# BGU-CS-VIL/DPMMSubClusters.jl

Hardware: NVIDIA B200
Metric: gibbs_iters_per_sec (higher is better)
Workload: dtype f32

## Files before the change

dpmmsubclusters.jl_b200/csrc/kernels_gauss_tc2.cuh:

```cuda
#pragma once
#include "tcgen05.cuh"
#include "kernels_gauss.cuh"
#include "kernels_stats.cuh"

#define T2_TILE 128
#define T2_PRODUCERS(D) ((D) == 32 ? 128 : 64)
#define T2_THREADS(D) (320 + T2_PRODUCERS(D))
#define T2_CMAX 8
#define T2_R 8
#define T2_DELTA 30.0f
#define T2_MAX_K 256
#define T2_COOP_MAX 12
#define T2_NS32 4

struct GaussTc2Args {
  const float* x;
  int64_t n;
  int K, KS, nch, n0;
  const int32_t* perm;
  const int32_t* seg_off;
  int nkeys;
  const float* wpiv;
  const float* wscr;
  const float* wbias;
// ... 489 lines not shown
            if constexpr (D == 64) {
              tc::tmem_ld32(taddr, v);
              tc::tmem_ld32(taddr + 32, v1);
              tc::tmem_ld_wait();
              qp = gauss_tc_screen_q(v) + gauss_tc_screen_q(v1);
            } else {
              tc::tmem_ld32(taddr, v);
              tc::tmem_ld32(taddr + 32, v1);
              tc::tmem_ld_wait();
              qp = gauss_tc_screen_q(v);
            }
            const float2 cf = ccfro[key];
            const float e = xnorm * cf.y;
            float sq;
            asm("sqrt.approx.ftz.f32 %0, %1;" : "=f"(sq) : "f"(fmaxf(qp, 0.f)));
            const float dr = fmaf(1.01f * sq, e, fmaf(0.5f * e, e, 0.01f));
            const float rt = fmaf(-0.5f, qp, cf.x);
            weird = !(fabsf(rt) < CUDART_INF_F) || !(dr < CUDART_INF_F);
            thr = (rt - dr) - T2_DELTA;
            A4 = 4.0816f * (0.01f - thr);
            A42 = f2_pack(A4, A4);
            col = D;
            if constexpr (D == 32) {
              uint32_t h = screen4(v1, 0);
              if ((unsigned)key < 4u) h &= ~(1u << key);
              if (h) append(h, 0);
              b0 = 1;
            }
          }
          for (; b0 < nb; b0 += 2) {
            uint32_t v[32], v1[32];
            tc::tmem_ld32(taddr + col + b0 * 32, v);
            if (b0 + 1 < nb) tc::tmem_ld32(taddr + col + b0 * 32 + 32, v1);
            tc::tmem_ld_wait();
            uint32_t h = screen4(v, c * 16 + b0 * 4);
            if (b0 + 1 < nb) h |= screen4(v1, c * 16 + b0 * 4 + 4) << 4;
            const int k0 = kbase + b0 * 4;
            if ((unsigned)(key - k0) < 8u) h &= ~(1u << (key - k0));
            if (h) append(h, k0);
          }
          tc::tc_fence_before();
          tc::mbar_arrive(&tempty[g * 2 + b]);
        }
        bool multi = valid && !weird && cnt > 0 && cnt < T2_CMAX;
        bool ovf = valid && (weird || cnt >= T2_CMAX);
        if (multi) {
          int j = cnt;
          while (j > 0 && mylist[j - 1] > key) {
            mylist[j] = mylist[j - 1];
            --j;
          }
          mylist[j] = (uint16_t)key;
          ++cnt;
        }
        if (__any_sync(0xffffffffu, multi)) {
          const int mine = multi ? cnt : 0;
          int inc = mine;
#pragma unroll
          for (int o = 1; o < 32; o <<= 1) {
            const int t = __shfl_up_sync(0xffffffffu, inc, o);
            if (lane >= o) inc += t;
          }
          const int total = __shfl_sync(0xffffffffu, inc, 31), off = inc - mine;
          uint16_t* wpairs = pairs + wq * 32 * T2_CMAX;
          for (int j = 0; j < mine; ++j) wpairs[off + j] = (uint16_t)((row << 3) | j);
          __syncwarp();
          if (total <= T2_COOP_MAX) {
            for (int p = 0; p < total; ++p) {
              const int pr = wpairs[p], prow = pr >> 3, slot = pr & 7;
              const int k = lists[prow * T2_CMAX + slot];
              const int32_t pidx = __ldg(a.perm + w.pos + prow);
              const float q = gauss_tc2_exact_q_coop<D>(a.urows + (size_t)k * D * D, a.mu + (size_t)k * D, a.x + (size_t)pidx * D, lane);
              if (lane == 0) {
                const float2 cf = cfin[k];
                rl[prow * T2_CMAX + slot] = gauss_finish(cf.x, q, cf.y);
                ++ncand_total;
              }
            }
          } else {
            for (int p = lane; p < total; p += 32) {
              const int pr = wpairs[p], prow = pr >> 3, slot = pr & 7;
              const int k = lists[prow * T2_CMAX + slot];
              const int32_t pidx = __ldg(a.perm + w.pos + prow);
              const float q = gauss_tc2_exact_q_row<D>(a.urows + (size_t)k * D * D, a.mu + (size_t)k * D, a.x + (size_t)pidx * D);
              const float2 cf = cfin[k];
              rl[prow * T2_CMAX + slot] = gauss_finish(cf.x, q, cf.y);
              ++ncand_total;
            }
          }
          __syncwarp();
        }
        tc::mbar_arrive(&empty[s]);
        if (valid) {
          int lab = key;
          if (multi) {
            bool bad = false;
            for (int j = 0; j < cnt; ++j) bad |= (myrl[j] != myrl[j]);
            if (bad) {
              ovf = true;
            } else if (a.final_iter) {
              float bv = -CUDART_INF_F;
              lab = mylist[0];
              for (int j = 0; j < cnt; ++j)
                if (myrl[j] > bv) {
                  bv = myrl[j];
                  lab = mylist[j];
                }
            } else {
              const double u = dpmm_uniform(a.u_inj, idx, a.seed, DPMM_STREAM_LABEL, a.call, (uint64_t)(a.goff + idx));
              lab = gauss_tc2_draw_list(mylist, myrl, cnt, K, u);
            }
          } else if (!ovf) {
            if (a.u_inj != nullptr && lab > 0 && !a.final_iter && a.u_inj[idx] == 0.0) lab = 0;
          }
          if (ovf) {
            a.ovf_list[atomicAdd(a.ovf_count, 1)] = idx;
          } else {
            a.labels[idx] = lab;
            atomicAdd(&hs[lab], 1);
          }
          ++npts_total;
        }
      }
      {
#pragma unroll
        for (int o = 16; o > 0; o >>= 1) {
          npts_total += __shfl_xor_sync(0xffffffffu, npts_total, o);
          ncand_total += __shfl_xor_sync(0xffffffffu, ncand_total, o);
        }
        if (lane == 0 && a.stats != nullptr) {
          atomicAdd(&a.stats[0], npts_total);
          atomicAdd(&a.stats[1], ncand_total);
        }
      }
    } else {
      const int t64 = tid - 320;
      constexpr int CPR = D / 4;
      constexpr int RS = T2_PRODUCERS(D) / CPR;
      constexpr int NJ = T2_TILE / RS;
      const int c = t64 % CPR, r0 = t64 / CPR;
      T2Walk wl, wc;
      t2_walk_init(wl, seq);
      wc = wl;
      int ckey = -1;
      float4 cen = make_float4(0.f, 0.f, 0.f, 0.f);
      int32_t idx[NJ];
      auto load_idx = [&]() {
#pragma unroll
        for (int j = 0; j < NJ; ++j) {
          const int p = wl.pos + r0 + RS * j;
          idx[j] = p < wl.end ? __ldg(a.perm + p) : -1;
        }
      };
      auto issue = [&](int s) {
        uint8_t* dst0 = stage0 + (size_t)s * L.stage_bytes + (c >> 3) * 16384;
#pragma unroll
        for (int j = 0; j < NJ; ++j) {
          const int r = r0 + RS * j;
          const bool ok = idx[j] >= 0;
          cp_async16(dst0 + r * 128 + (((c & 7) ^ (r & 7)) << 4), a.x + (size_t)(ok ? idx[j] : 0) * D + 4 * c, ok ? 16 : 0);
        }
      };
      load_idx();
#pragma unroll
      for (int q = 0; q < PF; ++q) {
        if (q < nt) {
          issue(q % NS);
          t2_advance(wl, seq);
          if (q + 1 < nt) load_idx();
        }
        cp_async_commit();
      }
      for (int li = 0; li < nt; ++li) {
        cp_async_wait_group<PF - 1>();
        {
          const int key = min(wc.key, K - 1);
          if (key != ckey) {
            ckey = key;
            cen = __ldg(reinterpret_cast<const float4*>(a.mu + (size_t)key * D) + c);
          }
          uint8_t* base = stage0 + (size_t)(li % NS) * L.stage_bytes + (c >> 3) * 16384;
          const int nrow = wc.end - wc.pos;
#pragma unroll
          for (int j = 0; j < NJ; ++j) {
            const int r = r0 + RS * j;
            float4* q = reinterpret_cast<float4*>(base + r * 128 + (((c & 7) ^ (r & 7)) << 4));
            float4 v = *q;
            if (r < nrow) {
              v.x -= cen.x; v.y -= cen.y; v.z -= cen.z; v.w -= cen.w;
              *q = v;
            }
          }
          t2_advance(wc, seq);
        }
        tc::fence_proxy_async();
        tc::mbar_arrive(&full[li % NS]);
        const int nx = li + PF;
        if (nx < nt) {
          tc::mbar_wait(&empty[nx % NS], ((nx / NS) & 1) ^ 1);
          issue(nx % NS);
          t2_advance(wl, seq);
          if (nx + 1 < nt) load_idx();
        }
        cp_async_commit();
      }
    }
  }
  tc::tc_fence_before();
  __syncthreads();
  if (warp == 1) tc::tmem_dealloc(tmem_base, 512);
  for (int k = tid; k < K; k += T2_THREADS(D))
    if (hs[k] != 0) atomicAdd(&a.hist[k], hs[k]);
}

struct GaussListArgs {
  const float* x;
  int K;
  const int32_t* list;
  const int32_t* count;
  const float* urows;
  const float* mu;
  const float* cst;
  const float* logw;
  int32_t* labels;
  int32_t* hist;
  const double* u_inj;
  uint64_t seed;
  uint32_t call;
  int64_t goff;
  int final_iter;
  int32_t* stats;
  int32_t* zero_next;
  int32_t* ticket;
  int scan_k;
  int32_t* seg_off;
  int32_t* scat_cursor;
  int32_t* lr_cursor;
};

template <int D>
__global__ void __launch_bounds__(256) gauss_label_list_kernel(const GaussListArgs a) {
  extern __shared__ float gl_rs[];
  const int lane = threadIdx.x & 31, wl = threadIdx.x >> 5;
  const int nlist = *a.count;
  if (a.zero_next != nullptr && blockIdx.x == 0 && threadIdx.x < 4) a.zero_next[threadIdx.x] = 0;
  float* rs = gl_rs + (size_t)wl * a.K;
  for (int e = blockIdx.x * 8 + wl; e < nlist; e += gridDim.x * 8) {
    const int32_t idx = a.list[e];
    const float* xr = a.x + (size_t)idx * D;
    for (int k = lane; k < a.K; k += 32) {
      const float q = gauss_tc2_exact_q_impl<D>(a.urows + (size_t)k * D * D, a.mu + (size_t)k * D,
                                                [&](int c) { return __ldg(reinterpret_cast<const float4*>(xr) + c); });
      rs[k] = gauss_finish(__ldg(a.cst + 3 * k), q, __ldg(a.logw + k));
    }
    __syncwarp();
    if (lane == 0) {
      int lab;
      if (a.final_iter) {
        lab = dpmm_draw_argmax(rs, 1, a.K);
      } else {
        const double u = dpmm_uniform(a.u_inj, idx, a.seed, DPMM_STREAM_LABEL, a.call, (uint64_t)(a.goff + idx));
        lab = dpmm_draw_inverse_cdf(rs, 1, a.K, u);
      }
      a.labels[idx] = lab;
      atomicAdd(a.hist + lab, 1);
      if (a.stats != nullptr) atomicAdd(&a.stats[1], a.K);
    }
    __syncwarp();
  }
  if (a.ticket != nullptr) {
    __shared__ int last_block;
    __shared__ int wtot[8];
    __threadfence();
    __syncthreads();
    if (threadIdx.x == 0) last_block = atomicAdd(a.ticket, 1) == (int)gridDim.x - 1;
    __syncthreads();
    if (last_block) {
      __threadfence();
      int carry = 0;
      for (int k0 = 0; k0 < a.scan_k; k0 += 256) {
        const int k = k0 + (int)threadIdx.x;
        const int v = k < a.scan_k ? __ldcg(a.hist + k) : 0;
        int inc = v;
#pragma unroll
        for (int o = 1; o < 32; o <<= 1) {
          const int t = __shfl_up_sync(0xffffffffu, inc, o);
          if (lane >= o) inc += t;
        }
        if (lane == 31) wtot[wl] = inc;
        __syncthreads();
        int before = 0, total = 0;
#pragma unroll
        for (int w = 0; w < 8; ++w) {
          before += w < wl ? wtot[w] : 0;
          total += wtot[w];
        }
        const int excl = carry + before + inc - v;
        if (k < a.scan_k) {
          a.seg_off[k] = excl;
          a.scat_cursor[k] = excl;
          a.lr_cursor[2 * k] = excl;
          a.lr_cursor[2 * k + 1] = excl + v;
        }
        carry += total;
        __syncthreads();
      }
      if (threadIdx.x == 0) {
        a.seg_off[a.scan_k] = carry;
        *a.ticket = 0;
      }
    }
  }
}
```

dpmmsubclusters.jl_b200/csrc/kernels_stats.cuh:

```cuda
#pragma once
#include "common.cuh"

struct StatsItem {
  int32_t key;
  int32_t begin;
  int32_t end;
};

#ifndef DPMM_TEMPLATES_ONLY
__global__ void stats_worklist_kernel(const int32_t* __restrict__ seg_off, const int32_t* __restrict__ lr_cursor,
                                      const uint8_t* __restrict__ wanted, int K, int chunk, StatsItem* items,
                                      int32_t* n_items, int32_t* next_item) {
  extern __shared__ int sc[];
  const int tid = threadIdx.x;
  for (int key = tid; key < 2 * K; key += blockDim.x) {
    const int k = key >> 1;
    int len = 0;
    if (wanted == nullptr || wanted[k]) {
      const int mid = lr_cursor[2 * k];
      len = (key & 1) ? seg_off[k + 1] - mid : mid - seg_off[k];
    }
    sc[key] = (len + chunk - 1) / chunk;
  }
  __syncthreads();
  if (tid == 0) {
    int run = 0;
    for (int key = 0; key < 2 * K; ++key) {
      const int c = sc[key];
      sc[key] = run;
      run += c;
    }
    *n_items = run;
    *next_item = 0;
  }
  __syncthreads();
  for (int key = tid; key < 2 * K; key += blockDim.x) {
    const int k = key >> 1;
    if (wanted != nullptr && !wanted[k]) continue;
    const int mid = lr_cursor[2 * k];
    const int b = (key & 1) ? mid : seg_off[k];
    const int e = (key & 1) ? seg_off[k + 1] : mid;
    int o = sc[key];
    for (int s = b; s < e; s += chunk) items[o++] = StatsItem{key, s, min(e, s + chunk)};
  }
}

#endif

template <int EP>
__device__ __forceinline__ void warp_transpose_reduce(float (&v)[EP], int lane) {
  static_assert(EP % 32 == 0, "EP must be a multiple of 32");
  int h = EP / 2;
#pragma unroll
  for (int s = 0; s < 5; ++s) {
    const int off = 16 >> s;
    const bool up = (lane & off) != 0;
#pragma unroll
    for (int e = 0; e < EP / 2; ++e) {
      if (e < h) {
        const float send = up ? v[e] : v[e + h];
        const float keep = up ? v[e + h] : v[e];
        v[e] = keep + __shfl_xor_sync(0xffffffffu, send, off);
      }
    }
    h >>= 1;
  }
}
template <int EP>
__device__ __forceinline__ int warp_transpose_entry(int lane, int j) {
  int e = j, h = EP / 2;
#pragma unroll
  for (int s = 0; s < 5; ++s) {
    if (lane & (16 >> s)) e += h;
    h >>= 1;
  }
  return e;
}

template <int D>
struct StatsCfg {
  static constexpr int BS = (D <= 8) ? D : 8;
  static constexpr int BSQ = (BS + 1) & ~1;
  static constexpr int NB = (D + BS - 1) / BS;
  static constexpr int NU = NB * (NB + 1) / 2;
  static constexpr int DPAD = NB * BS + (BSQ - BS);
  static constexpr bool VEC = (BS % 4 == 0);
  static constexpr int DS = VEC ? 4 * ((DPAD / 4) | 1) : ((DPAD & 1) ? DPAD : DPAD + 1);
  static constexpr int E = BS * BSQ;
  static constexpr int EP = (E + 31) / 32 * 32;
  static constexpr int G = (NU + 15) / 16;
  static constexpr int WPG = (NU + G - 1) / G;
  static constexpr int NS = (WPG >= 8) ? 1 : (8 / WPG);
  static constexpr int WARPS = WPG * NS;
  static constexpr int R = (NS >= 8) ? 2 : 4;
  static constexpr int TPTS = 32 * NS * R;
  static constexpr int STAGES = 4;
  static constexpr int MAX_CHUNK = 2048;
  static constexpr int SMEM_BYTES = STAGES * TPTS * DS * 4 + MAX_CHUNK * 4;
  static constexpr int MIN_CTAS = (WARPS * 32 <= 320) ? 2 : 1;
};

struct StatsArgs {
  const float* x;
  int D;
  const int32_t* perm2;
  const StatsItem* items;
  const int32_t* n_items;
  int32_t* next_item;
  double* acc;
  int rec;
};

__device__ __forceinline__ void cp_async16(void* smem_dst, const void* gmem_src, int src_bytes) {
  const unsigned d = (unsigned)__cvta_generic_to_shared(smem_dst);
  asm volatile("cp.async.cg.shared.global [%0], [%1], 16, %2;" ::"r"(d), "l"(gmem_src), "r"(src_bytes) : "memory");
}
__device__ __forceinline__ void cp_async4(void* smem_dst, const void* gmem_src, int src_bytes) {
  const unsigned d = (unsigned)__cvta_generic_to_shared(smem_dst);
  asm volatile("cp.async.ca.shared.global [%0], [%1], 4, %2;" ::"r"(d), "l"(gmem_src), "r"(src_bytes) : "memory");
}
__device__ __forceinline__ void cp_async_commit() { asm volatile("cp.async.commit_group;" ::: "memory"); }
__device__ __forceinline__ void cp_async_wait_all() { asm volatile("cp.async.wait_group 0;" ::: "memory"); }
template <int N>
__device__ __forceinline__ void cp_async_wait_group() { asm volatile("cp.async.wait_group %0;" ::"n"(N) : "memory"); }

template <int D>
__global__ void __launch_bounds__(StatsCfg<D>::WARPS * 32, StatsCfg<D>::MIN_CTAS)
niw_stats_kernel(const StatsArgs a) {
  using C = StatsCfg<D>;
  constexpr int BS = C::BS, BSQ = C::BSQ, NQ = C::BSQ / 2;
  extern __shared__ __align__(16) float xs_all[];
  int32_t* sidx = reinterpret_cast<int32_t*>(xs_all + C::STAGES * C::TPTS * C::DS);
  __shared__ int s_item;
  const int tid = threadIdx.x, lane = tid & 31, warp = tid >> 5;
  const int slice = warp / C::WPG;
  for (int e = tid; e < C::STAGES * C::TPTS * C::DS; e += blockDim.x) xs_all[e] = 0.f;

  auto prefetch = [&](const StatsItem& item, int t0, int buf) {
    float* xs = xs_all + buf * C::TPTS * C::DS;
    const int tn = min(C::TPTS, item.end - t0);
    const int32_t* ix = sidx + (t0 - item.begin);
    if constexpr (D % 4 == 0) {
      for (int e = tid; e < C::TPTS * (D / 4); e += blockDim.x) {
        const int p = e / (D / 4), c = e - p * (D / 4);
        const bool ok = p < tn;
        const int idx = ok ? ix[p] : 0;
        cp_async16(xs + p * C::DS + 4 * c, a.x + (size_t)idx * D + 4 * c, ok ? 16 : 0);
      }
    } else {
      for (int e = tid; e < C::TPTS * D; e += blockDim.x) {
        const int p = e / D, c = e - p * D;
        const bool ok = p < tn;
        const int idx = ok ? ix[p] : 0;
        cp_async4(xs + p * C::DS + c, a.x + (size_t)idx * D + c, ok ? 4 : 0);
      }
    }
    cp_async_commit();
  };

  for (;;) {
    __syncthreads();
    if (tid == 0) s_item = atomicAdd(a.next_item, 1);
    __syncthreads();
    const int it = s_item;
    if (it >= *a.n_items * C::G) break;
    const StatsItem item = a.items[it / C::G];
    for (int e = tid; e < item.end - item.begin; e += blockDim.x) sidx[e] = __ldg(a.perm2 + item.begin + e);
    __syncthreads();
    const int u = (it % C::G) * C::WPG + warp % C::WPG;
    const bool live = u < C::NU;
    int bi = 0, bj = 0;
    if (live) {
      int r = u;
      while (r >= C::NB - bi) {
        r -= C::NB - bi;
        ++bi;
      }
      bj = bi + r;
    }
    const bool diag = live && (bi == bj);
    f32x2_t acc[BS][NQ];
    float sx[BS];
#pragma unroll
    for (int p = 0; p < BS; ++p) {
      sx[p] = 0.f;
#pragma unroll
      for (int q = 0; q < NQ; ++q) acc[p][q] = 0ull;
    }

    const int ntl = (item.end - item.begin + C::TPTS - 1) / C::TPTS;
#pragma unroll
    for (int j = 0; j < C::STAGES - 1; ++j) {
      if (j < ntl) prefetch(item, item.begin + j * C::TPTS, j);
      else cp_async_commit();
    }
    for (int t = 0; t < ntl; ++t) {
      const int buf = t % C::STAGES;
      cp_async_wait_group<C::STAGES - 2>();
      __syncthreads();
      if (t + C::STAGES - 1 < ntl) prefetch(item, item.begin + (t + C::STAGES - 1) * C::TPTS, (t + C::STAGES - 1) % C::STAGES);
      else cp_async_commit();
      if (live) {
        const float* xs = xs_all + buf * C::TPTS * C::DS;
#pragma unroll
        for (int r = 0; r < C::R; ++r) {
          const float* row = xs + (slice * 32 * C::R + r * 32 + lane) * C::DS;
          float xi[BS];
          f32x2_t xj[NQ];
          if constexpr (C::VEC) {
#pragma unroll
            for (int q4 = 0; q4 < BS / 4; ++q4) {
              const float4 vi = *reinterpret_cast<const float4*>(row + bi * BS + 4 * q4);
              const ulonglong2 vj = *reinterpret_cast<const ulonglong2*>(row + bj * BS + 4 * q4);
              xi[4 * q4] = vi.x; xi[4 * q4 + 1] = vi.y; xi[4 * q4 + 2] = vi.z; xi[4 * q4 + 3] = vi.w;
              xj[2 * q4] = vj.x; xj[2 * q4 + 1] = vj.y;
            }
          } else {
#pragma unroll
            for (int q = 0; q < BS; ++q) xi[q] = row[bi * BS + q];
#pragma unroll
            for (int q = 0; q < NQ; ++q) xj[q] = f2_pack(row[bj * BS + 2 * q], row[bj * BS + 2 * q + 1]);
          }
#pragma unroll
          for (int p = 0; p < BS; ++p) {
            const f32x2_t xip = f2_pack(xi[p], xi[p]);
#pragma unroll
            for (int q = 0; q < NQ; ++q) acc[p][q] = f2_fma(xip, xj[q], acc[p][q]);
          }
          if (diag) {
#pragma unroll
            for (int p = 0; p < BS; ++p) sx[p] += xi[p];
          }
        }
      }
    }
    if (!live) continue;
    float accf[C::EP];
#pragma unroll
    for (int e = 0; e < C::EP; ++e) accf[e] = 0.f;
#pragma unroll
    for (int p = 0; p < BS; ++p)
#pragma unroll
      for (int q = 0; q < NQ; ++q) f2_unpack(acc[p][q], accf[p * BSQ + 2 * q], accf[p * BSQ + 2 * q + 1]);
    warp_transpose_reduce<C::EP>(accf, lane);
    double* dst = a.acc + (size_t)item.key * a.rec;
#pragma unroll
    for (int j = 0; j < C::EP / 32; ++j) {
      const int e = warp_transpose_entry<C::EP>(lane, j);
      if (e < C::E) {
        const int gi = bi * BS + e / BSQ, gj = bj * BS + e % BSQ;
        if (e % BSQ < BS && gi < D && gj < D && gi <= gj) atomicAdd(dst + 1 + D + (size_t)gi * D + gj, (double)accf[j]);
      }
    }
    if (diag) {
#pragma unroll
      for (int p = 0; p < BS; ++p) {
        float v = sx[p];
#pragma unroll
        for (int o = 16; o > 0; o >>= 1) v += __shfl_xor_sync(0xffffffffu, v, o);
        if (lane == p && bi * BS + p < D) atomicAdd(dst + 1 + bi * BS + p, (double)v);
      }
    }
  }
}

template <int D>
__global__ void __launch_bounds__(256) niw_stats_small_kernel(const StatsArgs a) {
  constexpr int NV = D + D * (D + 1) / 2;
  constexpr int NVP = (NV + 31) / 32 * 32;
  const int lane = threadIdx.x & 31;
  const int n_items = *a.n_items;
  for (;;) {
    int it = 0;
    if (lane == 0) it = atomicAdd(a.next_item, 1);
    it = __shfl_sync(0xffffffffu, it, 0);
    if (it >= n_items) break;
    const StatsItem item = a.items[it];
// ... 154 lines not shown
```

dpmmsubclusters.jl_b200/csrc/kernels_substats_tc.cuh:

```cuda
#pragma once
#include "kernels_gauss.cuh"
#include "kernels_stats_tc.cuh"

#define SS_D 32
#define SS_TILE 128
#define SS_RAW 5
#define SS_PF 2
#define SS_NG 3
#define SS_FLUSH 8
#define SS_NTB 6
#define SS_THREADS 896
#define SS_GATHER 256
#define SS_PANEL 16384
#define SS_PROWS 136
#define SS_PPANEL (SS_PROWS * 128)
#define SS_WSLOT (8192 + 8192 + 2048)
#define SS_TMEM_COLS 512
#define SS_TMEM_G2 (SS_NTB * 64)
#define SS_TLD 65

struct SubStatsArgs {
  const float* x;
  int64_t n;
  int K;
// ... 7 lines not shown
  uint8_t* sub;
  double* acc;
  int rec;
  int32_t* lcount;
  float* centers;
  const double* u_inj;
  uint64_t seed;
  uint32_t call;
  int64_t goff;
  float* dump;
};

struct SubStatsSmem {
  size_t raw, split, perm, wslot, aaug, tbuf, tri, dest, cnt, kcnt, bnd, pre, bars, slot, total;
  __host__ __device__ explicit SubStatsSmem(int K) {
    size_t o = 0;
    raw = o;    o += (size_t)SS_RAW * SS_PANEL;
    split = o;  o += (size_t)2 * SS_PANEL;
    perm = o;   o += (size_t)2 * 2 * SS_PPANEL;
    wslot = o;  o += (size_t)SS_WSLOT;
    aaug = o;   o += 4096;
    tbuf = o;   o += 64 * SS_TLD * 4;
    tri = o;    o += 528 * 2;
    o = (o + 15) & ~(size_t)15;
    dest = o;   o += SS_NG * SS_TILE;
    cnt = o;    o += SS_NG * 4 * 4;
    kcnt = o;   o += 4 * 4;
    bnd = o;    o += (size_t)(K + 1) * 4;
    pre = o;    o += (size_t)(K + 1) * 4;
    o = (o + 15) & ~(size_t)15;
    bars = o;   o += 40 * 8;
    slot = o;   o += 16;
    total = o;
  }
};

__global__ void __launch_bounds__(SS_THREADS, 1) niw_substats_tc_kernel(const SubStatsArgs a) {
  extern __shared__ __align__(1024) uint8_t ss_smem[];
  const SubStatsSmem L(a.K);
  uint8_t* raw0 = ss_smem + L.raw;
  uint8_t* split0 = ss_smem + L.split;
  uint8_t* perm0 = ss_smem + L.perm;
  uint8_t* wslot = ss_smem + L.wslot;
  float* aaug = reinterpret_cast<float*>(ss_smem + L.aaug);
  float* T = reinterpret_cast<float*>(ss_smem + L.tbuf);
  uint16_t* tri = reinterpret_cast<uint16_t*>(ss_smem + L.tri);
  uint8_t* dest_s = ss_smem + L.dest;
  volatile int32_t* cnt_s = reinterpret_cast<int32_t*>(ss_smem + L.cnt);
  volatile int32_t* kcnt = reinterpret_cast<int32_t*>(ss_smem + L.kcnt);
  int32_t* B = reinterpret_cast<int32_t*>(ss_smem + L.bnd);
  int32_t* P = reinterpret_cast<int32_t*>(ss_smem + L.pre);
  uint64_t* bars = reinterpret_cast<uint64_t*>(ss_smem + L.bars);
  uint64_t* ready = bars;
  uint64_t* sfree = bars + 2;
  uint64_t* landed = bars + 18;
  uint64_t* rfree = bars + 23;
  uint64_t* d1full = bars + 28;
  uint64_t* d1empty = bars + 34;
  uint64_t* permd = bars + 8;
  uint64_t* pfree = bars + 4;
  uint64_t* d2full = bars + 12;
  uint64_t* d2empty = bars + 14;
  uint64_t* wfull = bars + 16;
  uint64_t* wempty = bars + 17;
  uint32_t* tmem_slot = reinterpret_cast<uint32_t*>(ss_smem + L.slot);
  const int tid = threadIdx.x, lane = tid & 31, warp = tid >> 5;
  const int nkeys = a.K;

  for (int j = tid; j <= nkeys; j += SS_THREADS) B[j] = __ldg(a.seg_off + j);
  for (int e = tid; e < 1024; e += SS_THREADS) {
    const int i = e >> 5, j = e & 31;
    if (j >= i) tri[i * 32 - (i * (i - 1)) / 2 + (j - i)] = (uint16_t)((i << 8) | j);
  }
  for (int e = tid; e < 1024; e += SS_THREADS) aaug[e] = 0.f;
  {
    float* baug = reinterpret_cast<float*>(wslot + 16384);
    for (int e = tid; e < 512; e += SS_THREADS) baug[e] = 0.f;
  }
  if (blockIdx.x == 0)
    for (int e = tid; e < 2 * nkeys * SS_D; e += SS_THREADS)
      a.centers[e] = __ldg(a.cen + (size_t)(e >> 6) * SS_D + (e & 31));
  if (tid == 0) {
    for (int b = 0; b < SS_NTB; ++b) {
      tc::mbar_init(&d1full[b], 1);
      tc::mbar_init(&d1empty[b], 128);
    }
    for (int b = 0; b < 2; ++b) {
      tc::mbar_init(&permd[b], 128);
      tc::mbar_init(&d2full[b], 2);
      tc::mbar_init(&d2empty[b], 128);
    }
    for (int b = 0; b < 4; ++b) tc::mbar_init(&pfree[b], 2);
    for (int r = 0; r < SS_RAW; ++r) {
      tc::mbar_init(&landed[r], SS_GATHER);
      tc::mbar_init(&rfree[r], 128);
    }
    for (int b = 0; b < 2; ++b) {
      tc::mbar_init(&ready[b], SS_GATHER);
      tc::mbar_init(&sfree[b], 1);
    }
    tc::mbar_init(wfull, 32);
    tc::mbar_init(wempty, 1);
    tc::fence_barrier_init();
  }
  __syncthreads();
  for (int r = tid; r < SS_TILE; r += SS_THREADS) {
    float* p = aaug + (r >> 3) * 64 + (r & 7) * 4;
    p[0] = 1.f;
    p[1] = 1.f;
  }
  if (warp == 0) {
    int carry = 0;
    if (lane == 0) P[0] = 0;
    for (int base = 0; base < nkeys; base += 32) {
      const int j = base + lane;
      int v = j < nkeys ? (B[j + 1] - B[j] + SS_TILE - 1) / SS_TILE : 0;
#pragma unroll
      for (int o = 1; o < 32; o <<= 1) {
        const int u = __shfl_up_sync(0xffffffffu, v, o);
        if (lane >= o) v += u;
      }
      if (j < nkeys) P[j + 1] = carry + v;
      carry += __shfl_sync(0xffffffffu, v, 31);
    }
  }
  if (warp == 4) tc::tmem_alloc(tmem_slot, SS_TMEM_COLS);
  tc::fence_proxy_async();
  tc::tc_fence_before();
  __syncthreads();
  tc::tc_fence_after();
  const uint32_t tmem_base = *tmem_slot;
  const int ntot = P[nkeys];
  const int t0 = (int)(((int64_t)ntot * blockIdx.x) / gridDim.x);
  const int t1 = (int)(((int64_t)ntot * (blockIdx.x + 1)) / gridDim.x);
  const int nt = t1 - t0;

  if (nt > 0) {
    if (warp < 4 || (warp >= 19 && warp < 23)) {
      const int gtid = warp < 4 ? tid : tid - 608 + 128;
      const int c = gtid & 7, r0 = gtid >> 3;
      const uint32_t offk = (uint32_t)(r0 * 128 + ((c ^ (r0 & 7)) << 4));
      const uint32_t offr = offk;
      StcWalk wl, wc;
      stc_walk_init(wl, B, P, nkeys, t0, t1);
      wc = wl;
      int idx[4];
      auto load_idx = [&]() {
#pragma unroll
        for (int j = 0; j < 4; ++j) {
          const int p = wl.pos + r0 + 32 * j;
          idx[j] = p < wl.end ? __ldg(a.perm + p) : -1;
        }
      };
      auto issue = [&](int s) {
        uint8_t* dst = raw0 + (size_t)s * SS_PANEL + offr;
#pragma unroll
        for (int j = 0; j < 4; ++j) {
          const bool ok = idx[j] >= 0;
          cp_async16(dst + j * 4096, a.x + (size_t)(ok ? idx[j] : 0) * SS_D + 4 * c, ok ? 16 : 0);
        }
      };
#pragma unroll
      for (int li = 0; li < SS_PF; ++li) {
        if (li < nt) {
          load_idx();
          issue(li);
          stc_advance<SS_FLUSH>(wl, B);
        }
        cp_async_commit();
      }
      if (SS_PF < nt) load_idx();
      auto load_center = [&](int key) { return __ldg(reinterpret_cast<const float4*>(a.cen + (size_t)key * SS_D) + c); };
      int ckey = wc.key;
      float4 cen = load_center(ckey);
      for (int li = 0; li < nt; ++li) {
        const int b = li & 1;
        if (wc.key != ckey) {
          ckey = wc.key;
          cen = load_center(ckey);
        }
        const int npts = wc.end - wc.pos;
        cp_async_wait_group<SS_PF - 1>();
        uint8_t* src = raw0 + (size_t)(li % SS_RAW) * SS_PANEL + offr;
        float4 v[4];
#pragma unroll
        for (int j = 0; j < 4; ++j) v[j] = *reinterpret_cast<const float4*>(src + j * 4096);
        float4 lo[4];
#pragma unroll
        for (int j = 0; j < 4; ++j) {
          if (r0 + 32 * j < npts) {
            v[j].x -= cen.x; v[j].y -= cen.y; v[j].z -= cen.z; v[j].w -= cen.w;
          }
          *reinterpret_cast<float4*>(src + j * 4096) = v[j];
          lo[j].x = v[j].x - tc::trunc_tf32(v[j].x); lo[j].y = v[j].y - tc::trunc_tf32(v[j].y);
          lo[j].z = v[j].z - tc::trunc_tf32(v[j].z); lo[j].w = v[j].w - tc::trunc_tf32(v[j].w);
        }
        tc::mbar_arrive(&landed[li % SS_RAW]);
        tc::mbar_wait(&sfree[b], ((li >> 1) & 1) ^ 1);
        uint8_t* lk = split0 + (size_t)b * SS_PANEL + offk;
#pragma unroll
        for (int j = 0; j < 4; ++j) *reinterpret_cast<float4*>(lk + j * 4096) = lo[j];
        tc::fence_proxy_async();
        tc::mbar_arrive(&ready[b]);
        const int ln = li + SS_PF;
        if (ln < nt) {
          tc::mbar_wait(&rfree[ln % SS_RAW], ((ln / SS_RAW) & 1) ^ 1);
          issue(ln % SS_RAW);
          stc_advance<SS_FLUSH>(wl, B);
          if (ln + 1 < nt) load_idx();
        }
        cp_async_commit();
        stc_advance<SS_FLUSH>(wc, B);
      }
    } else if (warp == 4) {
      {
        const uint32_t tmem_u = __shfl_sync(0xffffffffu, tmem_base, 0);
        StcWalk wm;
        stc_walk_init(wm, B, P, nkeys, t0, t1);
        const uint32_t idesc1 = tc::idesc_tf32(64);
        const uint64_t aaug_desc = tc::smem_desc_k_noswz(tc::smem_u32(aaug));
        const uint32_t ws = tc::smem_u32(wslot);
        const uint64_t baug_desc = tc::smem_desc_k_noswz(ws + 16384);
        const uint64_t raw_desc = tc::smem_desc_k128(tc::smem_u32(raw0)), l_desc = tc::smem_desc_k128(tc::smem_u32(split0));
        uint64_t whd[4], wld[4];
#pragma unroll
        for (int ks = 0; ks < 4; ++ks) {
          whd[ks] = tc::smem_desc_k128(ws) + ks * 2;
          wld[ks] = tc::smem_desc_k128(ws + 8192) + ks * 2;
        }
        int kj = -1, prevkey = -1;
        for (int li = 0; li < nt; ++li) {
          const int b = li & 1;
          if (wm.key != prevkey) {
            prevkey = wm.key;
            ++kj;
            tc::mbar_wait(wfull, kj & 1);
          }
          const int tb = li % SS_NTB, tph = (li / SS_NTB) & 1;
          tc::mbar_wait(&ready[b], (li >> 1) & 1);
          tc::mbar_wait(&d1empty[tb], tph ^ 1);
          tc::tc_fence_after();
          uint64_t hd[4], ld[4];
#pragma unroll
          for (int ks = 0; ks < 4; ++ks) {
            hd[ks] = raw_desc + (uint64_t)((li % SS_RAW) * (SS_PANEL >> 4) + ks * 2);
            ld[ks] = l_desc + (uint64_t)(b * (SS_PANEL >> 4) + ks * 2);
          }
          const uint32_t tmem_d = tmem_u + tb * 64;
          tc::umma_tf32_first_w(tmem_d, hd[0], whd[0], idesc1);
#pragma unroll
          for (int ks = 1; ks < 4; ++ks) tc::umma_tf32_acc_w(tmem_d, hd[ks], whd[ks], idesc1);
#pragma unroll
          for (int ks = 0; ks < 4; ++ks) tc::umma_tf32_acc_w(tmem_d, ld[ks], whd[ks], idesc1);
#pragma unroll
          for (int ks = 0; ks < 4; ++ks) tc::umma_tf32_acc_w(tmem_d, hd[ks], wld[ks], idesc1);
          tc::umma_tf32_acc_w(tmem_d, aaug_desc, baug_desc, idesc1);
          tc::umma_commit_w(&sfree[b]);
          tc::umma_commit_w(&d1full[tb]);
          if (wm.pos + SS_TILE >= wm.end) tc::umma_commit_w(wempty);
          stc_advance<SS_FLUSH>(wm, B);
        }
      }
    } else if (warp == 18 || warp == 23) {
      {
        const int right = warp == 23 ? 1 : 0;
        const uint32_t tmem_u = __shfl_sync(0xffffffffu, tmem_base, 0);
        StcWalk wm;
        stc_walk_init(wm, B, P, nkeys, t0, t1);
        const uint32_t idesc2 = tc::idesc_tf32_mn_m64(32);
        const uint64_t pd0 = tc::smem_desc_mn128(tc::smem_u32(perm0), SS_PPANEL);
        const uint64_t pd1 = tc::smem_desc_mn128(tc::smem_u32(perm0 + 2 * SS_PPANEL), SS_PPANEL);
        int g2 = 0;
        for (int li = 0; li < nt; ++li) {
          const int b = li & 1;
          const bool first = wm.gcount == 0, last = stc_is_last<SS_FLUSH>(wm);
          tc::mbar_wait(&permd[b], (li >> 1) & 1);
          if (first) tc::mbar_wait(&d2empty[g2 & 1], ((g2 >> 1) & 1) ^ 1);
          tc::tc_fence_after();
          const int nkl = __shfl_sync(0xffffffffu, kcnt[b * 2], 0), nkr = __shfl_sync(0xffffffffu, kcnt[b * 2 + 1], 0);
          const int k0 = right ? nkl : 0, nk = right ? nkr : nkl;
          const uint32_t tm = tmem_u + SS_TMEM_G2 + (g2 & 1) * 64 + right * 32;
          uint64_t pd = (b ? pd1 : pd0) + (uint64_t)(k0 * 64);
          int ks = 0;
          if (first && nk > 0) {
            tc::umma_tf32_first_w(tm, pd, pd, idesc2);
            pd += 64;
            ks = 1;
          }
          for (; ks < nk; ++ks, pd += 64) tc::umma_tf32_acc_w(tm, pd, pd, idesc2);
          tc::umma_commit_w(&pfree[li & 3]);
          if (last) {
            tc::umma_commit_w(&d2full[g2 & 1]);
            ++g2;
          }
          stc_advance<SS_FLUSH>(wm, B);
        }
      }
    } else if (warp < 13 || warp >= 24) {
      const int g = warp >= 24 ? 2 + ((warp - 24) >> 2) : (warp - 5) >> 2;
      const int sub = warp & 3;
      const int row = (sub << 5) | lane;
      const int gt = warp >= 24 ? (tid - 768) & 127 : (tid - 160) & 127;
      uint8_t* const dest_g = dest_s + g * SS_TILE;
      volatile int32_t* const cnt_g = cnt_s + g * 4;
      int nacc = 0;
      const int c = gt & 7, r0 = gt >> 3;
      const uint32_t offr = (uint32_t)(r0 * 128 + ((c ^ (r0 & 7)) << 4));
      const uint32_t lt_mask = (1u << lane) - 1u;
      StcWalk we;
      stc_walk_init(we, B, P, nkeys, t0, t1);
      float sxl[4] = {0.f, 0.f, 0.f, 0.f}, sxr[4] = {0.f, 0.f, 0.f, 0.f};
      int ckey = -1;
      float cl = 0.f, cr = 0.f, lwl = 0.f, lwr = 0.f;
      for (int li = 0; li < nt; ++li) {
        if (li % SS_NG != g) {
          stc_advance<SS_FLUSH>(we, B);
          continue;
        }
        const int b = li & 1;
        const int key = we.key;
        const int npts = min(SS_TILE, we.end - we.pos);
        const bool valid = row < npts;
        const int32_t idx = valid ? __ldg(a.perm + we.pos + row) : 0;
        if (key != ckey) {
          ckey = key;
          cl = __ldg(a.cst + 3 * key + 1); cr = __ldg(a.cst + 3 * key + 2);
          lwl = __ldg(a.loglr + 2 * key); lwr = __ldg(a.loglr + 2 * key + 1);

        }
        double u = 0.0;
        if (valid) u = dpmm_uniform(a.u_inj, idx, a.seed, DPMM_STREAM_SUBLABEL, a.call, (uint64_t)(a.goff + idx));
        const int tb = li % SS_NTB;
        tc::mbar_wait(&d1full[tb], (li / SS_NTB) & 1);
        tc::tc_fence_after();
        uint32_t v0[32], v1[32];
        const uint32_t taddr = tmem_base + ((uint32_t)(sub * 32) << 16) + tb * 64;
        tc::tmem_ld32(taddr, v0);
        tc::tmem_ld32(taddr + 32, v1);
        tc::tmem_ld_wait();
        const float ql = gauss_tc_screen_q(v0), qr = gauss_tc_screen_q(v1);
        tc::tc_fence_before();
        tc::mbar_arrive(&d1empty[tb]);
        int side = 2;
        if (valid) {
          const float rl = gauss_finish(cl, ql, lwl), rr = gauss_finish(cr, qr, lwr);
          if (a.dump != nullptr) {
            a.dump[idx] = rl;
            a.dump[a.n + idx] = rr;
          }
          side = dpmm_draw_two(rl, rr, u);
          a.sub[idx] = (uint8_t)side;
        }
        const uint32_t bl = __ballot_sync(0xffffffffu, side == 0), br = __ballot_sync(0xffffffffu, side == 1);
        if (lane == 0) cnt_g[sub] = __popc(bl) | (__popc(br) << 8);
        asm volatile("bar.sync %0, 128;" ::"r"(1 + g) : "memory");
        int nl = 0, nr = 0, offl = 0, offr_ = 0;
#pragma unroll
        for (int w = 0; w < 4; ++w) {
          const int cw = cnt_g[w];
          if (w < sub) {
            offl += cw & 255;
            offr_ += cw >> 8;
          }
          nl += cw & 255;
          nr += cw >> 8;
// ... 163 lines not shown
```

Baseline: 5240.

## Gather rows into registers via non-caching loads instead of cp.async staging

For D=32 in the tcgen05 gauss kernel and in the substats kernel, producer warps now gather point rows straight into registers with ld.global.nc (L1 no_allocate), double-buffered across two register sets. They subtract the center in registers and write each value to the swizzled shared tile once. This removes the cp.async round trip (write to smem, read back, write again) and the wait-group stalls, and the empty/free barrier wait moves to just before the store. The cost is more register pressure and load latency exposed inside the producer warps, and in-flight depth is fixed at two tiles.

```diff
diff --git a/dpmmsubclusters.jl_b200/csrc/kernels_gauss_tc2.cuh b/dpmmsubclusters.jl_b200/csrc/kernels_gauss_tc2.cuh
--- a/dpmmsubclusters.jl_b200/csrc/kernels_gauss_tc2.cuh
+++ b/dpmmsubclusters.jl_b200/csrc/kernels_gauss_tc2.cuh
@@ -665,57 +665,112 @@
           idx[j] = p < wl.end ? __ldg(a.perm + p) : -1;
         }
       };
-      auto issue = [&](int s) {
-        uint8_t* dst0 = stage0 + (size_t)s * L.stage_bytes + (c >> 3) * 16384;
-#pragma unroll
-        for (int j = 0; j < NJ; ++j) {
-          const int r = r0 + RS * j;
-          const bool ok = idx[j] >= 0;
-          cp_async16(dst0 + r * 128 + (((c & 7) ^ (r & 7)) << 4), a.x + (size_t)(ok ? idx[j] : 0) * D + 4 * c, ok ? 16 : 0);
-        }
-      };
-      load_idx();
-#pragma unroll
-      for (int q = 0; q < PF; ++q) {
-        if (q < nt) {
-          issue(q % NS);
+      if constexpr (D == 32) {
+        static_assert(PF == 2, "one register set per tile in flight: va, vb");
+        auto load_rows = [&](float4 (&v)[NJ]) {
+#pragma unroll
+          for (int j = 0; j < NJ; ++j) {
+            const bool ok = idx[j] >= 0;
+            v[j] = ldg_nc16(a.x + (size_t)(ok ? idx[j] : 0) * D + 4 * c, ok);
+          }
+        };
+        float4 va[NJ], vb[NJ];
+        load_idx();
+        load_rows(va);
+        t2_advance(wl, seq);
+        if (1 < nt) {
+          load_idx();
+          load_rows(vb);
           t2_advance(wl, seq);
-          if (q + 1 < nt) load_idx();
-        }
-        cp_async_commit();
-      }
-      for (int li = 0; li < nt; ++li) {
-        cp_async_wait_group<PF - 1>();
-        {
+        }
+        if (2 < nt) load_idx();
+        auto tile = [&](int li, float4 (&v)[NJ]) {
           const int key = min(wc.key, K - 1);
           if (key != ckey) {
             ckey = key;
             cen = __ldg(reinterpret_cast<const float4*>(a.mu + (size_t)key * D) + c);
           }
-          uint8_t* base = stage0 + (size_t)(li % NS) * L.stage_bytes + (c >> 3) * 16384;
           const int nrow = wc.end - wc.pos;
+          t2_advance(wc, seq);
+#pragma unroll
+          for (int j = 0; j < NJ; ++j) {
+            if (r0 + RS * j < nrow) {
+              v[j].x -= cen.x; v[j].y -= cen.y; v[j].z -= cen.z; v[j].w -= cen.w;
+            }
+          }
+          tc::mbar_wait(&empty[li % NS], ((li / NS) & 1) ^ 1);
+          uint8_t* base = stage0 + (size_t)(li % NS) * L.stage_bytes;
 #pragma unroll
           for (int j = 0; j < NJ; ++j) {
             const int r = r0 + RS * j;
-            float4* q = reinterpret_cast<float4*>(base + r * 128 + (((c & 7) ^ (r & 7)) << 4));
-            float4 v = *q;
-            if (r < nrow) {
-              v.x -= cen.x; v.y -= cen.y; v.z -= cen.z; v.w -= cen.w;
-              *q = v;
-            }
-          }
-          t2_advance(wc, seq);
-        }
-        tc::fence_proxy_async();
-        tc::mbar_arrive(&full[li % NS]);
-        const int nx = li + PF;
-        if (nx < nt) {
-          tc::mbar_wait(&empty[nx % NS], ((nx / NS) & 1) ^ 1);
-          issue(nx % NS);
-          t2_advance(wl, seq);
-          if (nx + 1 < nt) load_idx();
-        }
-        cp_async_commit();
+            *reinterpret_cast<float4*>(base + r * 128 + ((c ^ (r & 7)) << 4)) = v[j];
+          }
+          tc::fence_proxy_async();
+          tc::mbar_arrive(&full[li % NS]);
+          const int nx = li + PF;
+          if (nx < nt) {
+            load_rows(v);
+            t2_advance(wl, seq);
+            if (nx + 1 < nt) load_idx();
+          }
+        };
+        for (int li = 0; li < nt; li += 2) {
+          tile(li, va);
+          if (li + 1 < nt) tile(li + 1, vb);
+        }
+      } else {
+        auto issue = [&](int s) {
+          uint8_t* dst0 = stage0 + (size_t)s * L.stage_bytes + (c >> 3) * 16384;
+#pragma unroll
+          for (int j = 0; j < NJ; ++j) {
+            const int r = r0 + RS * j;
+            const bool ok = idx[j] >= 0;
+            cp_async16(dst0 + r * 128 + (((c & 7) ^ (r & 7)) << 4), a.x + (size_t)(ok ? idx[j] : 0) * D + 4 * c, ok ? 16 : 0);
+          }
+        };
+        load_idx();
+#pragma unroll
+        for (int q = 0; q < PF; ++q) {
+          if (q < nt) {
+            issue(q % NS);
+            t2_advance(wl, seq);
+            if (q + 1 < nt) load_idx();
+          }
+          cp_async_commit();
+        }
+        for (int li = 0; li < nt; ++li) {
+          cp_async_wait_group<PF - 1>();
+          {
+            const int key = min(wc.key, K - 1);
+            if (key != ckey) {
+              ckey = key;
+              cen = __ldg(reinterpret_cast<const float4*>(a.mu + (size_t)key * D) + c);
+            }
+            uint8_t* base = stage0 + (size_t)(li % NS) * L.stage_bytes + (c >> 3) * 16384;
+            const int nrow = wc.end - wc.pos;
+#pragma unroll
+            for (int j = 0; j < NJ; ++j) {
+              const int r = r0 + RS * j;
+              float4* q = reinterpret_cast<float4*>(base + r * 128 + (((c & 7) ^ (r & 7)) << 4));
+              float4 v = *q;
+              if (r < nrow) {
+                v.x -= cen.x; v.y -= cen.y; v.z -= cen.z; v.w -= cen.w;
+                *q = v;
+              }
+            }
+            t2_advance(wc, seq);
+          }
+          tc::fence_proxy_async();
+          tc::mbar_arrive(&full[li % NS]);
+          const int nx = li + PF;
+          if (nx < nt) {
+            tc::mbar_wait(&empty[nx % NS], ((nx / NS) & 1) ^ 1);
+            issue(nx % NS);
+            t2_advance(wl, seq);
+            if (nx + 1 < nt) load_idx();
+          }
+          cp_async_commit();
+        }
       }
     }
   }
diff --git a/dpmmsubclusters.jl_b200/csrc/kernels_stats.cuh b/dpmmsubclusters.jl_b200/csrc/kernels_stats.cuh
--- a/dpmmsubclusters.jl_b200/csrc/kernels_stats.cuh
+++ b/dpmmsubclusters.jl_b200/csrc/kernels_stats.cuh
@@ -123,6 +123,15 @@
 __device__ __forceinline__ void cp_async_wait_all() { asm volatile("cp.async.wait_group 0;" ::: "memory"); }
 template <int N>
 __device__ __forceinline__ void cp_async_wait_group() { asm volatile("cp.async.wait_group %0;" ::"n"(N) : "memory"); }
+__device__ __forceinline__ float4 ldg_nc16(const void* gmem_src, bool ok) {
+  float4 v;
+  asm volatile("{\n .reg .pred p;\n setp.ne.b32 p, %5, 0;\n"
+               " mov.f32 %0, 0f00000000; mov.f32 %1, 0f00000000; mov.f32 %2, 0f00000000; mov.f32 %3, 0f00000000;\n"
+               " @p ld.global.nc.L1::no_allocate.v4.f32 {%0, %1, %2, %3}, [%4];\n}"
+               : "=f"(v.x), "=f"(v.y), "=f"(v.z), "=f"(v.w)
+               : "l"(gmem_src), "r"((int)ok));
+  return v;
+}
 
 template <int D>
 __global__ void __launch_bounds__(StatsCfg<D>::WARPS * 32, StatsCfg<D>::MIN_CTAS)
diff --git a/dpmmsubclusters.jl_b200/csrc/kernels_substats_tc.cuh b/dpmmsubclusters.jl_b200/csrc/kernels_substats_tc.cuh
--- a/dpmmsubclusters.jl_b200/csrc/kernels_substats_tc.cuh
+++ b/dpmmsubclusters.jl_b200/csrc/kernels_substats_tc.cuh
@@ -183,65 +183,67 @@
           idx[j] = p < wl.end ? __ldg(a.perm + p) : -1;
         }
       };
-      auto issue = [&](int s) {
-        uint8_t* dst = raw0 + (size_t)s * SS_PANEL + offr;
+      auto load_rows = [&](float4 (&v)[4]) {
 #pragma unroll
         for (int j = 0; j < 4; ++j) {
           const bool ok = idx[j] >= 0;
-          cp_async16(dst + j * 4096, a.x + (size_t)(ok ? idx[j] : 0) * SS_D + 4 * c, ok ? 16 : 0);
+          v[j] = ldg_nc16(a.x + (size_t)(ok ? idx[j] : 0) * SS_D + 4 * c, ok);
         }
       };
-#pragma unroll
-      for (int li = 0; li < SS_PF; ++li) {
-        if (li < nt) {
-          load_idx();
-          issue(li);
-          stc_advance<SS_FLUSH>(wl, B);
-        }
-        cp_async_commit();
+      float4 va[4], vb[4];
+      load_idx();
+      load_rows(va);
+      stc_advance<SS_FLUSH>(wl, B);
+      if (1 < nt) {
+        load_idx();
+        load_rows(vb);
+        stc_advance<SS_FLUSH>(wl, B);
       }
       if (SS_PF < nt) load_idx();
       auto load_center = [&](int key) { return __ldg(reinterpret_cast<const float4*>(a.cen + (size_t)key * SS_D) + c); };
       int ckey = wc.key;
       float4 cen = load_center(ckey);
-      for (int li = 0; li < nt; ++li) {
+      auto tile = [&](int li, float4 (&v)[4]) {
         const int b = li & 1;
         if (wc.key != ckey) {
           ckey = wc.key;
           cen = load_center(ckey);
         }
         const int npts = wc.end - wc.pos;
-        cp_async_wait_group<SS_PF - 1>();
-        uint8_t* src = raw0 + (size_t)(li % SS_RAW) * SS_PANEL + offr;
-        float4 v[4];
-#pragma unroll
-        for (int j = 0; j < 4; ++j) v[j] = *reinterpret_cast<const float4*>(src + j * 4096);
-        float4 lo[4];
 #pragma unroll
         for (int j = 0; j < 4; ++j) {
           if (r0 + 32 * j < npts) {
             v[j].x -= cen.x; v[j].y -= cen.y; v[j].z -= cen.z; v[j].w -= cen.w;
           }
-          *reinterpret_cast<float4*>(src + j * 4096) = v[j];
-          lo[j].x = v[j].x - tc::trunc_tf32(v[j].x); lo[j].y = v[j].y - tc::trunc_tf32(v[j].y);
-          lo[j].z = v[j].z - tc::trunc_tf32(v[j].z); lo[j].w = v[j].w - tc::trunc_tf32(v[j].w);
-        }
+        }
+        tc::mbar_wait(&rfree[li % SS_RAW], ((li / SS_RAW) & 1) ^ 1);
+        uint8_t* zk = raw0 + (size_t)(li % SS_RAW) * SS_PANEL + offr;
+#pragma unroll
+        for (int j = 0; j < 4; ++j) *reinterpret_cast<float4*>(zk + j * 4096) = v[j];
         tc::mbar_arrive(&landed[li % SS_RAW]);
         tc::mbar_wait(&sfree[b], ((li >> 1) & 1) ^ 1);
         uint8_t* lk = split0 + (size_t)b * SS_PANEL + offk;
 #pragma unroll
-        for (int j = 0; j < 4; ++j) *reinterpret_cast<float4*>(lk + j * 4096) = lo[j];
+        for (int j = 0; j < 4; ++j) {
+          float4 lo;
+          lo.x = v[j].x - tc::trunc_tf32(v[j].x); lo.y = v[j].y - tc::trunc_tf32(v[j].y);
+          lo.z = v[j].z - tc::trunc_tf32(v[j].z); lo.w = v[j].w - tc::trunc_tf32(v[j].w);
+          *reinterpret_cast<float4*>(lk + j * 4096) = lo;
+        }
         tc::fence_proxy_async();
         tc::mbar_arrive(&ready[b]);
         const int ln = li + SS_PF;
         if (ln < nt) {
-          tc::mbar_wait(&rfree[ln % SS_RAW], ((ln / SS_RAW) & 1) ^ 1);
-          issue(ln % SS_RAW);
+          load_rows(v);
           stc_advance<SS_FLUSH>(wl, B);
           if (ln + 1 < nt) load_idx();
         }
-        cp_async_commit();
         stc_advance<SS_FLUSH>(wc, B);
+      };
+      static_assert(SS_PF == 2, "one register set per tile in flight: va, vb");
+      for (int li = 0; li < nt; li += 2) {
+        tile(li, va);
+        if (li + 1 < nt) tile(li + 1, vb);
       }
     } else if (warp == 4) {
       {
```

Result: faster. 5407, median of 6 (+3.2%).
